# suutari/meterelf

Measured on AMD Instinct MI355X. Metric: frames/sec (640x480), full pipeline, digits identical to the oracle, higher is better.
Workload: dtype u8; 1 GPU; Batch=1024 per GPU, full pipeline incl. TM_CCOEFF match + needle reading, 4 dials/frame, sample-images1 params, frames 480x640 synthesised from the readable fixtures (shift +-8, noise sigma 2), 4 distinct batches in rotation (3.77 GB of frames per GPU); global_batch=1024, parallelism=dp1, frames_read_ok_batch0=1023

## Files before the change

### meterelf_amd/csrc/k_match_mfma.hip

```cpp
#include <limits.h>
#include <stdio.h>
#include <stdlib.h>
#include <string.h>

#include <algorithm>

#include "melf_device.h"
#include <hip/hip_ext.h>

#include "melf_internal.h"

namespace melf {

typedef int i32x4 __attribute__((ext_vector_type(4)));
typedef int i32x8 __attribute__((ext_vector_type(8)));
typedef int i32x16 __attribute__((ext_vector_type(16)));

typedef unsigned int u32x4m __attribute__((ext_vector_type(4)));

typedef uint32_t u32x4a4 __attribute__((ext_vector_type(4), aligned(4)));
template <bool FROM_BGR>
__global__ __launch_bounds__(256) void k_prep_lplane(MatchSrc src, int nframes, int nkb, int rows_pad, int tw, int rwp, int pairs,
                                                     int8_t* __restrict__ Lg, uint16_t* __restrict__ R)
{
    constexpr int PX = FROM_BGR ? 3 : 1;
#include "prep_lplane_body.inc"
}

__global__ __launch_bounds__(256) void k_lplane_px4(MatchSrc src, int nframes, int nkb, int rows_pad, int tw, int rwp, int pairs,
                                                    int8_t* __restrict__ Lg, uint16_t* __restrict__ R)
{
    constexpr int PX = 4;
#include "prep_lplane_body.inc"
}

struct MfmaGeom {
    int rh, rw;
    int rows_pad;
    int th_pad;
    int nframes;
    int nparts;
    int na;
    int k1;
    int rows, th;
    int ntiles;
    double tmean;
};

#ifdef MELF_MATCH_STAMP
__device__ uint64_t g_match_stamps[4 * 8192];
__device__ uint64_t g_match_loop_end[8192];
extern "C" __attribute__((visibility("default"))) int melf_debug_match_stamps(uint64_t* out, int nwaves)
{
    return hipMemcpyFromSymbol(out, HIP_SYMBOL(g_match_stamps), sizeof(uint64_t) * 4 * (size_t)(nwaves < 8192 ? nwaves : 8192)) == hipSuccess ? 0 : -1;
}
extern "C" __attribute__((visibility("default"))) int melf_debug_match_loop_end(uint64_t* out, int nwaves)
{
    return hipMemcpyFromSymbol(out, HIP_SYMBOL(g_match_loop_end), sizeof(uint64_t) * (size_t)(nwaves < 8192 ? nwaves : 8192)) == hipSuccess ? 0 : -1;
}
#endif

__device__ inline bool better_m(float v, int i, float bv, int bi)
{
    return i != INT_MAX && (bi == INT_MAX || v > bv || (v == bv && i < bi));
}

template <int R, int NXB, int KS>
struct SliceLds {
    uint32_t acc[R * NXB][16][64];
    uint32_t wsa[32][64];
};

constexpr int MM_NF_DEV = 8;
template <int ND, int NXB, int R, int PD , int MFIRST, int MLAST, int KS = 1>
__device__ __forceinline__ void match_wave(const int8_t* __restrict__ Lg, const int8_t* __restrict__ Atab,
                                           const uint32_t* __restrict__ ws, const MfmaGeom& g,
                                           float* __restrict__ result_map, MatchPartial* __restrict__ partials,
                                           int grp, int rblk, int y0, void* lds_raw = nullptr)
{
    auto on = [](int r, int xb) -> bool {
        return r == 0 ? ((MFIRST >> xb) & 1) : (r == R - 1 ? ((MLAST >> xb) & 1) : true);
    };
    constexpr int NKB = ND + NXB - 1;
    constexpr int NBUF = R + PD;
    static_assert(PD == 1, "the template fragments are single-buffered: the next row's fragment d is requested right after this row's last use of fragment d");
    const int lane = threadIdx.x & 63;
    const int ks = KS > 1 ? __builtin_amdgcn_readfirstlane((int)(threadIdx.x >> 6)) : 0;
    const int SL = g.th_pad / KS, i_lo = ks * SL, i_hi = i_lo + SL;
    auto mine = [&](int r) -> bool { return KS == 1 || (r * KS) / R == ks; };
    SliceLds<R, NXB, KS>* const X = (SliceLds<R, NXB, KS>*)lds_raw;
    if (KS > 1) {
        uint32_t* z = (uint32_t*)X;
        for (int i = threadIdx.x; i < (int)(sizeof(SliceLds<R, NXB, KS>) / 4); i += 64 * KS) z[i] = 0;
        __syncthreads();
    }

    const uint32_t l16 = (uint32_t)lane * 16u;
    const __amdgpu_buffer_rsrc_t rsL = __builtin_amdgcn_make_buffer_rsrc(const_cast<int8_t*>(Lg + (size_t)grp * g.rows_pad * (size_t)NKB * 1024), 0,
                                                                         (int)((unsigned)g.rows_pad * (unsigned)NKB * 1024u), 0x27000);
    const __amdgpu_buffer_rsrc_t rsA = __builtin_amdgcn_make_buffer_rsrc(const_cast<int8_t*>(Atab + 1024), 0, (int)((unsigned)(g.th_pad + PD) * MM_NF_DEV * 1024u), 0x27000);
    const unsigned rsR_bytes = (unsigned)g.rows * 4096u;
    const __amdgpu_buffer_rsrc_t rsR = __builtin_amdgcn_make_buffer_rsrc(const_cast<uint32_t*>(ws + (size_t)grp * g.rows * 1024), 0, (int)rsR_bytes, 0x27000);
    auto LD = [&](__amdgpu_buffer_rsrc_t rs, unsigned rowoff, int slot) -> i32x4 {
        return __builtin_amdgcn_raw_buffer_load_b128(rs, l16, rowoff + (unsigned)slot * 1024u, 0);
    };
    const unsigned Lrow = (unsigned)y0 * (unsigned)NKB * 1024u;
    const int idxP = ((const int*)Atab)[lane];
    const int idxLo = 0x44444444, idxHi = (int)0xEEEEEEEEu;
    constexpr unsigned ROWB = (unsigned)NKB * 1024u;
    constexpr unsigned AROWB = (unsigned)MM_NF_DEV * 1024u;
    constexpr int NP = NXB;
    constexpr int NKD = NKB - 2 * NP;
    static_assert(ND == 7 && (NXB == 1 || NXB == 2), "the sub-block schedule below is written out for 7 Toeplitz blocks");

    i32x16 acc[R][NXB];
#pragma unroll
    for (int r = 0; r < R; ++r)
#pragma unroll
        for (int xb = 0; xb < NXB; ++xb)
#pragma unroll
            for (int e = 0; e < 16; ++e) acc[r][xb][e] = 0;

    constexpr int PERIOD = NBUF;
    const int istart = i_lo + (((SL - y0 % SL) % SL) / PERIOD) * PERIOD;
    i32x8 pp[NBUF][NP];
    i32x4 kd[NBUF][NKD];
    i32x4 a06, ad[5], a1s, a5s;
    uint32_t wsa[32];
    i32x4 rwv[4];
    auto rw_row = [&](int i) -> unsigned {
        return i < g.th ? (unsigned)min(y0 + i, g.rows - 1) * 4096u : rsR_bytes;
    };
    auto load_pp = [&](i32x8& d, unsigned row, int slot) {
        const i32x4 lo = LD(rsL, row, slot), hi = LD(rsL, row, slot + 1);
        d = __builtin_shufflevector(lo, hi, 0, 1, 2, 3, 4, 5, 6, 7);
    };
    auto SP = [&](int r, int xb, const i32x4& a, const i32x8& b, int idx) {
        if (on(r, xb)) acc[r][xb] = __builtin_amdgcn_smfmac_i32_32x32x64_i8(a, b, acc[r][xb], idx, 0, 0);
    };
    auto DN = [&](int r, int xb, const i32x4& a, const i32x4& b) {
        if (on(r, xb)) acc[r][xb] = __builtin_amdgcn_mfma_i32_32x32x32_i8(a, b, acc[r][xb], 0, 0, 0);
    };
    constexpr int NM1_0 = R - ((MFIRST & 1) == 0) - ((MLAST & 1) == 0);
    constexpr int NM1_1 = NXB == 2 ? R - ((MFIRST & 2) == 0) - ((MLAST & 2) == 0) : 0;
    constexpr int NM2 = NM1_0 + NM1_1;
#pragma unroll
    for (int j = 0; j < 32; ++j) wsa[j] = 0;
    auto ws_add = [&](int p) {
#pragma unroll
        for (int c = 0; c < 4; ++c) {
            const uint32_t v = (uint32_t)rwv[p][c];
            wsa[8 * p + 2 * c] += v & 0xffffu;
            wsa[8 * p + 2 * c + 1] += v >> 16;
            asm("" : "+v"(wsa[8 * p + 2 * c]));
            asm("" : "+v"(wsa[8 * p + 2 * c + 1]));
        }
    };
#define MELF_SGB(MFMAS, VALUS) __builtin_amdgcn_sched_group_barrier(0x008, MFMAS, 0); __builtin_amdgcn_sched_group_barrier(0x002, VALUS, 0);
#define MELF_SPREAD(NM) \
    if constexpr ((NM) >= 8) { MELF_SGB(1, 1) MELF_SGB(1, 1) MELF_SGB(1, 1) MELF_SGB(1, 1) MELF_SGB(1, 1) MELF_SGB(1, 1) MELF_SGB(1, 1) MELF_SGB(1, 1) } \
    else if constexpr ((NM) >= 4) { MELF_SGB(1, 2) MELF_SGB(1, 2) MELF_SGB(1, 2) MELF_SGB(1, 2) } \
    else { MELF_SGB(1, 4) MELF_SGB(1, 4) }
#define MELF_FENCE __builtin_amdgcn_sched_barrier(0);
#define MELF_LOAD1 __builtin_amdgcn_sched_group_barrier(0x008, 1, 0); __builtin_amdgcn_sched_group_barrier(0x020, 1, 0);
#define MELF_LOADS1 MELF_LOAD1
#define MELF_LOADS2 MELF_LOAD1 MELF_LOAD1
#define MELF_LOADS3 MELF_LOAD1 MELF_LOAD1 MELF_LOAD1
    for (int phase = 0; phase < 2; ++phase) {
        const int ibeg = phase == 0 ? istart : i_lo, iend = phase == 0 ? i_hi : istart;
        if (ibeg >= iend) continue;
#pragma unroll
        for (int r = 0; r < NBUF - 1; ++r) {
            const unsigned row = Lrow + (unsigned)(ibeg + r) * ROWB;
#pragma unroll
            for (int p = 0; p < NP; ++p) load_pp(pp[r][p], row, 2 * p);
#pragma unroll
            for (int c = 0; c < NKD; ++c) kd[r][c] = LD(rsL, row, 2 * NP + c);
        }
        {
            const unsigned an = (unsigned)ibeg * AROWB;
            a06 = LD(rsA, an, 0);
#pragma unroll
            for (int d = 0; d < 5; ++d) ad[d] = LD(rsA, an, 1 + d);
            if constexpr (NXB == 2) { a1s = LD(rsA, an, 6); a5s = LD(rsA, an, 7); }
            const unsigned rp = rw_row(ibeg);
#pragma unroll
            for (int k = 0; k < 4; ++k) rwv[k] = LD(rsR, rp, k);
        }
        for (int i0 = ibeg; i0 < iend; i0 += PERIOD) {
#pragma unroll
            for (int s = 0; s < PERIOD; ++s) {
                const int i = i0 + s;
                const unsigned rowin = Lrow + (unsigned)(i + NBUF - 1) * ROWB;
                const unsigned an = (unsigned)(i + 1) * AROWB;
                const unsigned rwn = rw_row(i + 1);
                const int inc = (s + NBUF - 1) % NBUF;
#define CUR(r) ((s + (r)) % NBUF)
                if constexpr (NXB == 2) {
                    const unsigned rowinp = rowin - ROWB, anc = (unsigned)i * AROWB;
                    const int incp = (s + NBUF - 2) % NBUF;
                    MELF_FENCE
                    ad[4] = LD(rsA, anc, 5);
                    kd[incp][3] = LD(rsL, rowinp, 7);
#pragma unroll
                    for (int r = 0; r < R; ++r) { SP(r, 0, a06, pp[CUR(r)][0], idxP); SP(r, 1, a06, pp[CUR(r)][1], idxP); }
                    ws_add(0);
                    MELF_LOADS2 MELF_SPREAD(NM2 - 2)
                    MELF_FENCE
                    a06 = LD(rsA, an, 0);
                    rwv[0] = LD(rsR, rwn, 0);
#pragma unroll
                    for (int r = 0; r < R; ++r) SP(r, 1, a5s, pp[CUR(r)][0], idxHi);
                    MELF_LOADS2
                    MELF_FENCE
                    a5s = LD(rsA, an, 7);
                    load_pp(pp[inc][0], rowin, 0);
#pragma unroll
                    for (int r = 0; r < R; ++r) SP(r, 0, a1s, pp[CUR(r)][1], idxLo);
                    MELF_LOADS3
                    MELF_FENCE
                    a1s = LD(rsA, an, 6);
                    load_pp(pp[inc][1], rowin, 2);
#pragma unroll
                    for (int r = 0; r < R; ++r) DN(r, 1, ad[0], kd[CUR(r)][0]);
                    MELF_LOADS3
#pragma unroll
                    for (int q = 0; q < 3; ++q) {
                        MELF_FENCE
                        ad[q] = LD(rsA, an, 1 + q);
                        if (q >= 1) { kd[inc][q - 1] = LD(rsL, rowin, 4 + q - 1); rwv[q] = LD(rsR, rwn, q); }
#pragma unroll
                        for (int r = 0; r < R; ++r) { DN(r, 0, ad[1 + q], kd[CUR(r)][q]); DN(r, 1, ad[1 + q], kd[CUR(r)][q + 1]); }
                        ws_add(1 + q);
                        if (q >= 1) { MELF_LOADS3 MELF_SPREAD(NM2 - 3) } else { MELF_LOADS1 MELF_SPREAD(NM2 - 1) }
                    }
                    MELF_FENCE
                    ad[3] = LD(rsA, an, 4);
                    kd[inc][2] = LD(rsL, rowin, 6);
                    rwv[3] = LD(rsR, rwn, 3);
#pragma unroll
                    for (int r = 0; r < R; ++r) DN(r, 0, ad[4], kd[CUR(r)][3]);
                    MELF_LOADS3
                    MELF_FENCE
                } else {
                    MELF_FENCE
#pragma unroll
                    for (int r = 0; r < R; ++r) SP(r, 0, a06, pp[CUR(r)][0], idxP);
                    ws_add(0);
                    MELF_SPREAD(NM1_0)
                    MELF_FENCE
                    a06 = LD(rsA, an, 0);
#pragma unroll
                    for (int d = 0; d < 5; ++d) {
                        if (d == 0) load_pp(pp[inc][0], rowin, 0);
                        else kd[inc][d - 1] = LD(rsL, rowin, 2 + d - 1);
                        if (d < 4) rwv[d] = LD(rsR, rwn, d);
                        MELF_FENCE
#pragma unroll
                        for (int r = 0; r < R; ++r) DN(r, 0, ad[d], kd[CUR(r)][d]);
                        if (d < 3) { ws_add(1 + d); MELF_SPREAD(NM1_0) }
                        MELF_FENCE
                        ad[d] = LD(rsA, an, 1 + d);
                    }
                    kd[inc][4] = LD(rsL, rowin, 6);
                    MELF_FENCE
                }
#undef CUR
            }
        }
    }
#undef MELF_SGB
#undef MELF_SPREAD
#undef MELF_FENCE
#undef MELF_LOAD1
#undef MELF_LOADS1
#undef MELF_LOADS2
#undef MELF_LOADS3

#ifdef MELF_MATCH_STAMP
    if (threadIdx.x == 0 && blockIdx.x < 8192) g_match_loop_end[blockIdx.x] = __builtin_amdgcn_s_memtime();
#endif
    if constexpr (KS > 1) {
#pragma unroll
        for (int j = 0; j < 32; ++j) __hip_atomic_fetch_add(&X->wsa[j][lane], wsa[j], __ATOMIC_RELAXED, __HIP_MEMORY_SCOPE_WORKGROUP);
#pragma unroll
        for (int r = 0; r < R; ++r)
#pragma unroll
            for (int xb = 0; xb < NXB; ++xb) {
                if (!on(r, xb)) continue;
                if (!mine(r)) {
#pragma unroll
                    for (int e = 0; e < 16; ++e)
                        __hip_atomic_fetch_add(&X->acc[r * NXB + xb][e][lane], (uint32_t)acc[r][xb][e], __ATOMIC_RELAXED, __HIP_MEMORY_SCOPE_WORKGROUP);
                }
            }
        __syncthreads();
#pragma unroll
        for (int j = 0; j < 32; ++j) wsa[j] = X->wsa[j][lane];
#pragma unroll
        for (int r = 0; r < R; ++r)
#pragma unroll
            for (int xb = 0; xb < NXB; ++xb) {
                if (!on(r, xb)) continue;
                if (mine(r)) {
#pragma unroll
                    for (int e = 0; e < 16; ++e) acc[r][xb][e] += (int)X->acc[r * NXB + xb][e][lane];
                }
            }
    }
    const int n = lane & 31, hh = lane >> 5;
    const int f = grp * 32 + n;
    const bool lane_ok = f < g.nframes;
    float bestv = -INFINITY;
    int bestc = -1;
    i32x4 slide[2][4];
    auto slide_load = [&](int r) {
        const unsigned rout = (unsigned)min(y0 + r - 1, g.rows - 1) * 4096u;
        const unsigned rin = (unsigned)min(y0 + r - 1 + g.th, g.rows - 1) * 4096u;
#pragma unroll
        for (int k = 0; k < 4; ++k) { slide[0][k] = LD(rsR, rout, k); slide[1][k] = LD(rsR, rin, k); }
    };
#pragma unroll
    for (int r = 0; r < R; ++r) {
        if (r > 0) {
#pragma unroll
            for (int k = 0; k < 4; ++k)
#pragma unroll
                for (int c = 0; c < 4; ++c) {
                    const uint32_t a0 = (uint32_t)slide[1][k][c], b0 = (uint32_t)slide[0][k][c];
                    wsa[8 * k + 2 * c] += (a0 & 0xffffu) - (b0 & 0xffffu);
                    wsa[8 * k + 2 * c + 1] += (a0 >> 16) - (b0 >> 16);
                }
        }
        if (r + 1 < R) slide_load(r + 1);
        __builtin_amdgcn_sched_barrier(0);
        if (!mine(r)) continue;
        const int y = y0 + r;
        if (y >= g.rh) continue;
        float v[NXB][16];
#pragma unroll
        for (int xb = 0; xb < NXB; ++xb)
#pragma unroll
            for (int e = 0; e < 16; ++e) {
                if (!on(r, xb)) continue;
                const uint32_t wsv = wsa[16 * xb + e];
                const uint32_t cc = (uint32_t)acc[r][xb][e] + 128u * wsv + (uint32_t)g.k1;
                double num = (double)cc;
                num -= (double)wsv * g.tmean;
                v[xb][e] = (float)num;
            }
#pragma unroll
        for (int xb = 0; xb < NXB; ++xb) {
            if (!on(r, xb) || 32 * xb + 32 <= g.rw) continue;
#pragma unroll
            for (int e = 0; e < 16; ++e)
                if (32 * xb + (e & 3) + 8 * (e >> 2) + 4 * hh >= g.rw) v[xb][e] = -INFINITY;
        }
#pragma unroll
        for (int xb = 0; xb < NXB; ++xb)
#pragma unroll
            for (int e = 0; e < 16; ++e) {
                if (!on(r, xb)) continue;
                if (v[xb][e] > bestv) { bestv = v[xb][e]; bestc = (r * NXB + xb) * 16 + e; }
            }
        if (result_map) {
            float* mrow = result_map + (size_t)f * g.rh * g.rw + (size_t)y * g.rw;
#pragma unroll
            for (int xb = 0; xb < NXB; ++xb)
#pragma unroll
                for (int e = 0; e < 16; ++e) {
                    if (!on(r, xb)) continue;
                    const int x = 32 * xb + (e & 3) + 8 * (e >> 2) + 4 * hh;
                    if (lane_ok && x < g.rw) mrow[x] = v[xb][e];
                }
        }
        __builtin_amdgcn_sched_barrier(0);
    }
    int besti = INT_MAX;
    if (bestc >= 0) {
        const int e = bestc & 15, xb = (bestc >> 4) % NXB, r = (bestc >> 4) / NXB;
        besti = (y0 + r) * g.rw + 32 * xb + (e & 3) + 8 * (e >> 2) + 4 * hh;
    }
    {
        const float ov = __shfl_xor(bestv, 32, 64);
        const int oi = __shfl_xor(besti, 32, 64);
        if (better_m(ov, oi, bestv, besti)) { bestv = ov; besti = oi; }
    }
    if (lane < 32 && f < g.nframes) {
        MatchPartial p;
        p.val = bestv;
        p.idx = besti;
        partials[(size_t)f * g.nparts + rblk * KS + ks] = p;
    }
}


template <int ND, int NXB, int RB, int PD, int KS>
__device__ __forceinline__ void match_block(const int8_t* __restrict__ Lg, const int8_t* __restrict__ Atab,
                                            const uint32_t* __restrict__ ws, const MfmaGeom& g,
                                            float* __restrict__ result_map, MatchPartial* __restrict__ partials, void* lds)
{
    const int nblk = gridDim.x;
    const int id = blockIdx.x;
#ifdef MELF_MATCH_STAMP
    const uint64_t st_clk = __builtin_amdgcn_s_memtime(), st_rt = __builtin_amdgcn_s_memrealtime();
#endif
    const int per = nblk / 8, rem = nblk % 8, xcd = id & 7, sub = id >> 3;
    const int vid = (xcd < rem ? xcd * (per + 1) : rem * (per + 1) + (xcd - rem) * per) + sub;
    const int grp = vid / g.ntiles, rblk = vid - grp * g.ntiles;
    if (NXB == 2 && RB < 5 && rblk >= g.na) {
        const int q = rblk - g.na, base = RB * g.na + (2 * RB + 1) * (q >> 1);
        if ((q & 1) == 0) match_wave<ND, 2, (RB < 5 ? RB + 1 : RB), PD, 3, 1, KS>(Lg, Atab, ws, g, result_map, partials, grp, rblk, base, lds);
        else match_wave<ND, 2, (RB < 5 ? RB + 1 : RB), PD, 2, 3, KS>(Lg, Atab, ws, g, result_map, partials, grp, rblk, base + RB, lds);
    } else {
        match_wave<ND, NXB, RB, PD, 3, 3, KS>(Lg, Atab, ws, g, result_map, partials, grp, rblk, rblk * RB, lds);
    }
#ifdef MELF_MATCH_STAMP
    if (threadIdx.x == 0 && id < 8192) {
        g_match_stamps[4 * id + 0] = st_clk; g_match_stamps[4 * id + 1] = __builtin_amdgcn_s_memtime();
        g_match_stamps[4 * id + 2] = st_rt;  g_match_stamps[4 * id + 3] = __builtin_amdgcn_s_memrealtime();
    }
#endif
}

template <int ND, int NXB, int RB, int PD, int KS = 1>
__global__ __launch_bounds__(64 * KS, 1) void k_match_mfma(const int8_t* __restrict__ Lg, const int8_t* __restrict__ Atab,
                                                           const uint32_t* __restrict__ ws, MfmaGeom g,
                                                           float* __restrict__ result_map, MatchPartial* __restrict__ partials)
{
    if constexpr (NXB == 2 && RB >= 4) asm volatile("" ::: "a199");
    if constexpr (KS > 1) {
        __shared__ __attribute__((aligned(16))) SliceLds<(NXB == 2 && RB < 5 ? RB + 1 : RB), NXB, KS> lds;
        match_block<ND, NXB, RB, PD, KS>(Lg, Atab, ws, g, result_map, partials, &lds);
    } else {
        match_block<ND, NXB, RB, PD, 1>(Lg, Atab, ws, g, result_map, partials, nullptr);
    }
}
constexpr int MM_ND = 7, MM_PD = 1;
constexpr int MM_NF = 8;
static int round_up(int v, int m) { return (v + m - 1) / m * m; }
static int mm_th_pad(int th, int rb, bool pairs, int ks = 1)
{
    static const int lcm2[6] = {0, 0, 12, 20, 30, 6};
    return ks * round_up((th + ks - 1) / ks, pairs ? lcm2[rb] : rb + 1);
}
static int mm_th_pad_max(int th) { return std::max(round_up(th, 60), std::max(mm_th_pad(th, 4, true, 2), mm_th_pad(th, 4, true, 4))); }

bool mfma_match_ok(int th, int tw, int rows, int cols)
{
    const int rh = rows - th + 1, rw = cols - tw + 1;
    const int nd = (tw + 31 + 31) / 32;
    return rh >= 1 && rw >= 1 && rw <= 64 && nd == MM_ND && tw <= 32 * (MM_ND - 1) && cols <= 32 * (MM_ND + (rw > 32 ? 2 : 1) - 1) &&
           (long)th * tw * 65025L < (1L << 32);
}

static double mm_wave_cycles(int R, int units, int nxb, int th_pad, int ks = 1)
{
    const int nkb = MM_ND + nxb - 1;
    const int nf = nxb == 2 ? 8 : 6;
    const double load = R >= 4 ? 7.0 : (R == 3 ? 17.0 : 30.0);
    return (double)(th_pad / ks) * ((double)units * (MM_ND - 1) * 32.0 + (double)(nkb + nf + 4) * load) + (double)((units + ks - 1) / ks) * 1300.0 + 4000.0 + R * 300.0 +
           (ks > 1 ? 6000.0 : 0.0);
}

MfmaPlan mfma_plan(int th, int tw, int rows, int cols, int nframes)
{
    MfmaPlan p = {};
    p.rh = rows - th + 1;
    p.rw = cols - tw + 1;
    p.nxb = p.rw > 32 ? 2 : 1;
    p.nkb = MM_ND + p.nxb - 1;
    p.groups = (nframes + 31) / 32;
    const int simds = 1024;
    int force_rb = 0, force_np = -1, force_ks = 0;
    if (const char* e = getenv("MELF_MATCH_LAYOUT")) {
        if (sscanf(e, "%d,%d,%d", &force_rb, &force_np, &force_ks) < 1 || force_rb < 2 || force_rb > 5) { force_rb = 0; force_np = -1; force_ks = 0; }
        if (force_ks != 1 && force_ks != 2 && force_ks != 4) force_ks = force_rb ? 1 : 0;
        if (force_ks > 1 && force_rb != 4) force_ks = 1;
    }
    double best = 0;
    p.rb = 0;
    p.ks = 1;
    for (int ks = 1; ks <= 4; ks *= 2) {
        if (force_ks && ks != force_ks) continue;
        for (int rb = 2; rb <= 5; ++rb) {
            if (force_rb && rb != force_rb) continue;
            if (ks > 1 && rb != 4) continue;
            const int np_max = (p.nxb == 2 && rb < 5) ? (p.rh + 2 * rb) / (2 * rb + 1) : 0;
            auto waves_of = [&](int np) -> long {
                const int rest = p.rh - (2 * rb + 1) * np;
                return (long)((rest > 0 ? (rest + rb - 1) / rb : 0) + 2 * np) * p.groups * ks;
            };
            long rounds_min = LONG_MAX;
            for (int np = 0; np <= np_max; ++np) rounds_min = std::min(rounds_min, (waves_of(np) + simds - 1) / simds);
            int np_few = 0;
            while (np_few < np_max && (waves_of(np_few) + simds - 1) / simds > rounds_min) ++np_few;
            for (int np = 0; np <= np_max; ++np) {
                if (force_np >= 0) { if (np != std::min(force_np, np_max)) continue; }
                else if (np != 0 && np != np_few) continue;
                const int rest = p.rh - (2 * rb + 1) * np;
                const int na = rest > 0 ? (rest + rb - 1) / rb : 0;
                const long waves = (long)(na + 2 * np) * p.groups * ks;
                const long rounds = (waves + simds - 1) / simds;
                const int th_pad = mm_th_pad(th, rb, np > 0, ks);
                const int upr = p.nxb;
                const double w_full = mm_wave_cycles(rb, upr * rb, p.nxb, th_pad, ks), w_pair = mm_wave_cycles(rb + 1, upr * rb + 1, p.nxb, th_pad, ks);
                const double longest = np > 0 ? w_pair : w_full;
                const double total = (double)p.groups * ks * ((double)na * w_full + 2.0 * np * w_pair);
                const double w_avg = total / (double)std::max<long>(waves, 1);
                const long full = waves / simds, part = waves - full * simds;
                const double cost = (double)full * 1.5 * w_avg + (part > 0 ? std::max(longest, 1.5 * (double)part * w_avg / simds) : 0.0);
                (void)rounds;
                if (!p.rb || cost < best * 0.98) {
                    best = cost;
                    p.rb = rb; p.na = na; p.np = np; p.th_pad = th_pad; p.ks = ks;
                }
            }
        }
    }
    p.ntiles = p.na + 2 * p.np;
    p.nparts = p.ntiles * p.ks;
    const int rows_cov = p.rb * p.na + (2 * p.rb + 1) * p.np;
    p.rows_pad = rows_cov + p.th_pad + MM_PD + 1;
    p.lg_bytes = (size_t)p.groups * p.rows_pad * p.nkb * 1024;
    p.r_bytes = (size_t)p.groups * rows * 64 * 32 * sizeof(uint16_t);
    return p;
}

size_t mfma_atab_bytes(int th)
{
    return 1024 + (size_t)(mm_th_pad_max(th) + MM_PD) * MM_NF * 1024;
}

void mfma_build_atab(const uint8_t* templ, int th, int tw, int8_t* atab)
{
    const int th_pad = mm_th_pad_max(th);
    uint32_t* idx = (uint32_t*)atab;
    memset(atab, 0, 1024);
    int8_t* fr = atab + 1024;
    auto cand_cols = [&](int m, int hA, int ja, int cols[4]) {
        const int hB = ja >> 3, t = 4 * hA + ((ja >> 1) & 3), k0 = 16 * hB + 2 * t;
        cols[0] = k0 - m; cols[1] = k0 + 1 - m; cols[2] = 32 * (MM_ND - 1) + k0 - m; cols[3] = cols[2] + 1;
        return k0;
    };
    int pos[64][16];
    for (int l = 0; l < 64; ++l)
        for (int ja = 0; ja < 16; ja += 2) {
            int cols[4], cand[4], nc = 0;
            cand_cols(l & 31, l >> 5, ja, cols);
            for (int v = 0; v < 4; ++v) if (cols[v] >= 0 && cols[v] < tw) cand[nc++] = v;
            if (nc > 2) { fprintf(stderr, "[melf] mfma_build_atab: template of %d columns does not pair up\n", tw); abort(); }
            int v0 = 0, v1 = 1;
            if (nc == 2) { v0 = cand[0]; v1 = cand[1]; }
            else if (nc == 1) { v0 = cand[0] < 3 ? cand[0] : 0; v1 = 3; }
            pos[l][ja] = v0; pos[l][ja + 1] = v1;
            idx[l] |= ((uint32_t)v0 << (2 * ja)) | ((uint32_t)v1 << (2 * ja + 2));
        }
    for (int i = 0; i < th_pad + MM_PD; ++i) {
        auto Tq = [&](int col) -> int8_t { return (i < th && col >= 0 && col < tw) ? (int8_t)((int)templ[(size_t)i * tw + col] - 128) : (int8_t)0; };
        int8_t* row = fr + (size_t)i * MM_NF * 1024;
        for (int l = 0; l < 64; ++l) {
            const int m = l & 31, hA = l >> 5;
            for (int d = 1; d <= 5; ++d)
                for (int j = 0; j < 16; ++j) row[((size_t)d * 64 + l) * 16 + j] = Tq(32 * d + 16 * hA + j - m);
            for (int ja = 0; ja < 16; ++ja) {
                int cols[4];
                const int k0 = cand_cols(m, hA, ja & ~1, cols);
                row[((size_t)0 * 64 + l) * 16 + ja] = Tq(cols[pos[l][ja]]);
                row[((size_t)6 * 64 + l) * 16 + ja] = Tq(32 * 1 + k0 + (ja & 1) - m);
                row[((size_t)7 * 64 + l) * 16 + ja] = Tq(32 * 5 + k0 + (ja & 1) - m);
            }
        }
    }
}

void launch_match_prep(const MatchSrc& src, int pix, int n, int groups, int rows_pad, int nkb, int rwp, int tw, int8_t* d_lg,
                       uint16_t* d_r, hipStream_t stream, int pairs)
{
    dim3 grid(rows_pad, groups), block(256);
    const size_t pre_bytes = (size_t)32 * (nkb * 32 + 8) * sizeof(int16_t);
    int dev = 0;
    (void)hipGetDevice(&dev);
    static bool attr_set[64] = {false};
    if (dev >= 0 && dev < 64 && !attr_set[dev]) {
        (void)hipFuncSetAttribute((const void*)k_prep_lplane<true>, hipFuncAttributeMaxDynamicSharedMemorySize, 128 * 1024);
        (void)hipFuncSetAttribute((const void*)k_prep_lplane<false>, hipFuncAttributeMaxDynamicSharedMemorySize, 128 * 1024);
        (void)hipFuncSetAttribute((const void*)k_lplane_px4, hipFuncAttributeMaxDynamicSharedMemorySize, 128 * 1024);
        attr_set[dev] = true;
    }
    if (pix == PIX_PLANE) hipLaunchKernelGGL((k_prep_lplane<false>), grid, block, pre_bytes, stream, src, n, nkb, rows_pad, tw, rwp, pairs, d_lg, d_r);
    else if (pix_bytes(pix) == 4) hipLaunchKernelGGL(k_lplane_px4, grid, block, pre_bytes, stream, src, n, nkb, rows_pad, tw, rwp, pairs, d_lg, d_r);
    else hipLaunchKernelGGL((k_prep_lplane<true>), grid, block, pre_bytes, stream, src, n, nkb, rows_pad, tw, rwp, pairs, d_lg, d_r);
}

void launch_mfma_prep(const MatchSrc& src, int pix, int n, const MfmaPlan& p, int th, int tw, int8_t* d_lg,
                      uint16_t* d_r, hipStream_t stream)
{
    (void)th;
    launch_match_prep(src, pix, n, p.groups, p.rows_pad, p.nkb, 64, tw, d_lg, d_r, stream, p.nxb);
}

template <int NXB, int RB, int KS>
static void launch_mm(dim3 grid, hipStream_t stream, hipEvent_t ev_start, hipEvent_t ev_stop, const int8_t* d_lg,
                      const int8_t* d_atab, const uint32_t* d_ws, const MfmaGeom& g, float* d_result_map, MatchPartial* d_partials)
{
    hipExtLaunchKernelGGL((k_match_mfma<MM_ND, NXB, RB, MM_PD, KS>), grid, dim3(64 * KS), 0, stream, ev_start, ev_stop, 0, d_lg, d_atab, d_ws, g,
                              d_result_map, d_partials);
}

void launch_mfma_match(int n, const MfmaPlan& p, int th, int tw, long tsum, double tmean, const int8_t* d_atab,
                       const int8_t* d_lg, const uint32_t* d_ws, float* d_result_map, MatchPartial* d_partials,
                       hipStream_t stream, hipEvent_t ev_start, hipEvent_t ev_stop)
{
    MfmaGeom g;
    g.rh = p.rh; g.rw = p.rw; g.rows_pad = p.rows_pad; g.th_pad = p.th_pad; g.nframes = n; g.nparts = p.nparts;
    g.na = p.na; g.ntiles = p.ntiles;
    g.k1 = (int)(128 * (tsum - 128L * th * tw));
    g.rows = p.rh + th - 1; g.th = th;
    g.tmean = tmean;
    dim3 grid(p.ntiles * p.groups);
#define MM_CASE(NXB_, RB_) \
    case NXB_ * 8 + RB_: launch_mm<NXB_, RB_, 1>(grid, stream, ev_start, ev_stop, d_lg, d_atab, d_ws, g, d_result_map, d_partials); break;
#define MM_CASE_KS(NXB_, KS_) \
    case 64 * KS_ + NXB_ * 8 + 4: launch_mm<NXB_, 4, KS_>(grid, stream, ev_start, ev_stop, d_lg, d_atab, d_ws, g, d_result_map, d_partials); break;
    switch ((p.ks > 1 ? 64 * p.ks : 0) + p.nxb * 8 + p.rb) {
        MM_CASE(1, 2) MM_CASE(1, 3) MM_CASE(1, 4) MM_CASE(1, 5)
        MM_CASE(2, 2) MM_CASE(2, 3) MM_CASE(2, 4) MM_CASE(2, 5)
        MM_CASE_KS(1, 2) MM_CASE_KS(2, 2) MM_CASE_KS(1, 4) MM_CASE_KS(2, 4)
        default:
            fprintf(stderr, "[melf] k_match_mfma: no instantiation for %d column blocks x %d rows per wave x %d K slices\n", p.nxb, p.rb, p.ks);
            abort();
    }
#undef MM_CASE
#undef MM_CASE_KS
}

}
```

### meterelf_amd/csrc/prep_lplane_body.inc

```
    constexpr int PB = PX == 4 ? 4 : 3;
    constexpr int WIN = PX == 4 ? 128 : 100;
    __shared__ __attribute__((aligned(16))) uint32_t tile[8 * 2 * 32 * 4];
    extern __shared__ int16_t pre_dyn[];
    const int pstride = nkb * 32 + 8;
    const int y = blockIdx.x, grp = blockIdx.y;
    const int t = threadIdx.x, n = t >> 3, kl = t & 7;
    const int f = grp * 32 + n;
    int carry = 0;
    const bool rows_safe = (size_t)min(grp * 32 + 31, nframes - 1) * src.frame_stride + (size_t)(src.y0 + y) * src.row_stride +
                           (size_t)(src.x0 + 32 * (nkb - 1)) * PB + WIN <= src.readable;
    u32x4m* out = (u32x4m*)(Lg + ((size_t)grp * rows_pad + y) * (size_t)nkb * 1024);
    for (int kc = 0; kc < nkb; kc += 8) {
        const int kb = kc + kl;
        uint32_t w[8] = {0, 0, 0, 0, 0, 0, 0, 0};
        const bool live = kb < nkb && f < nframes && y < src.rows && kb * 32 < src.cols;
        if (live) {
            const uint8_t* prow = src.base + (size_t)f * src.frame_stride + (size_t)(src.y0 + y) * src.row_stride;
            const int xbeg = kb * 32;
            const int npx = min(32, src.cols - xbeg);
            if (PX == 3) {
                const size_t o = (size_t)(src.x0 + xbeg) * 3;
                const uint8_t* p = prow + o;
                const int mis = (int)((size_t)p & 3);
                if (rows_safe || (size_t)f * src.frame_stride + (size_t)(src.y0 + y) * src.row_stride + o + 100 <= src.readable) {
                    const uint32_t* q = (const uint32_t*)(p - mis);
                    uint32_t d[25];
#pragma unroll
                    for (int i = 0; i < 25; ++i) d[i] = q[i];
                    uint32_t a[24];
#pragma unroll
                    for (int i = 0; i < 24; ++i) a[i] = __builtin_amdgcn_alignbit(d[i + 1], d[i], (uint32_t)mis * 8u);
#pragma unroll
                    for (int k = 0; k < 32; ++k) {
                        const int j = (3 * k) >> 2, sh = ((3 * k) & 3) * 8;
                        const uint32_t px = sh <= 8 ? (a[j] >> sh) : __builtin_amdgcn_alignbit(a[j + 1 < 24 ? j + 1 : 23], a[j], sh);
                        const int L = hls_lightness_fast(px & 255, (px >> 8) & 255, (px >> 16) & 255);
                        w[k >> 2] |= (uint32_t)((L - 128) & 255) << ((k & 3) * 8);
                    }
                } else {
                    for (int k = 0; k < npx; ++k) {
                        const int L = hls_lightness(p[3 * k], p[3 * k + 1], p[3 * k + 2]);
                        w[k >> 2] |= (uint32_t)((L - 128) & 255) << ((k & 3) * 8);
                    }
                }
            } else if (PX == 4) {
                const size_t o = (size_t)(src.x0 + xbeg) * 4;
                const uint8_t* p = prow + o;
                if (rows_safe || (size_t)f * src.frame_stride + (size_t)(src.y0 + y) * src.row_stride + o + 128 <= src.readable) {
                    const u32x4a4* q = (const u32x4a4*)p;
                    u32x4a4 d[8];
#pragma unroll
                    for (int i = 0; i < 8; ++i) d[i] = q[i];
#pragma unroll
                    for (int k = 0; k < 32; ++k) {
                        const uint32_t px = d[k >> 2][k & 3];
                        const int L = hls_lightness_fast(px & 255, (px >> 8) & 255, (px >> 16) & 255);
                        w[k >> 2] |= (uint32_t)((L - 128) & 255) << ((k & 3) * 8);
                    }
                } else {
                    for (int k = 0; k < npx; ++k) {
                        const uint32_t px = ((const uint32_t*)p)[k];
                        const int L = hls_lightness(px & 255, (px >> 8) & 255, (px >> 16) & 255);
                        w[k >> 2] |= (uint32_t)((L - 128) & 255) << ((k & 3) * 8);
                    }
                }
            } else {
                const uint8_t* p = prow + src.x0 + xbeg;
                for (int k = 0; k < npx; ++k) w[k >> 2] |= (uint32_t)(((int)p[k] - 128) & 255) << ((k & 3) * 8);
            }
        }
        if (kc) __syncthreads();
#pragma unroll
        for (int h = 0; h < 2; ++h) {
            u32x4m v = {w[4 * h], w[4 * h + 1], w[4 * h + 2], w[4 * h + 3]};
            *(u32x4m*)(tile + ((kl * 2 + h) * 32 + n) * 4) = v;
        }
        int run = 0;
#pragma unroll
        for (int j = 0; j < 8; ++j) run = __builtin_amdgcn_sdot4((int)w[j], 0x01010101, run, false);
        int off = run;
#pragma unroll
        for (int dlt = 1; dlt < 8; dlt <<= 1) {
            const int o2 = __shfl_up(off, dlt, 8);
            if (kl >= dlt) off += o2;
        }
        const int chunk_total = __shfl(off, 7, 8);
        off += carry - run;
        carry += chunk_total;
        if (kb < nkb) {
            int acc = off;
#pragma unroll
            for (int k = 0; k < 32; k += 2) {
                acc += (int)(int8_t)((w[k >> 2] >> ((k & 3) * 8)) & 255u);
                const uint32_t lo16 = (uint32_t)acc & 0xffffu;
                acc += (int)(int8_t)((w[k >> 2] >> (((k + 1) & 3) * 8)) & 255u);
                *(uint32_t*)&pre_dyn[n * pstride + kb * 32 + k] = lo16 | ((uint32_t)acc << 16);
            }
        }
        __syncthreads();
        const int nb = min(8, nkb - kc);
        if (pairs == 0) {
            for (int i = t; i < nb * 64; i += 256) out[kc * 64 + i] = *(const u32x4m*)(tile + i * 4);
        } else {
            for (int i = t; i < nb * 64; i += 256) {
                const int slot = i >> 6, li = i & 63;
                u32x4m v;
                if (slot < 2 * pairs) {
                    const int p = slot >> 1, hl = slot & 1;
                    const uint2 lo2 = *(const uint2*)(tile + (p * 64 + li) * 4 + 2 * hl), hi2 = *(const uint2*)(tile + ((p + 6) * 64 + li) * 4 + 2 * hl);
                    v.x = __builtin_amdgcn_perm(hi2.x, lo2.x, 0x05040100u); v.y = __builtin_amdgcn_perm(hi2.x, lo2.x, 0x07060302u);
                    v.z = __builtin_amdgcn_perm(hi2.y, lo2.y, 0x05040100u); v.w = __builtin_amdgcn_perm(hi2.y, lo2.y, 0x07060302u);
                } else {
                    v = *(const u32x4m*)(tile + ((slot - pairs) * 64 + li) * 4);
                }
                out[i] = v;
            }
        }
    }
    if (y < src.rows) {
        uint16_t* ro = R + (((size_t)grp * src.rows + y) * rwp) * 32;
        const int bias = tw * 128;
        const int pmax = nkb * 32 - 1;
        const int ln = t & 63, nn = ln & 31, hh = ln >> 5;
        for (int kk = t >> 6; kk < rwp / 16; kk += 4) {
            const int xb = kk >> 1, e0 = 8 * (kk & 1);
            uint32_t o[4];
#pragma unroll
            for (int q = 0; q < 8; ++q) {
                const int e = e0 + q;
                const int x = 32 * xb + (e & 3) + 8 * (e >> 2) + 4 * hh;
                const int hi = (int)pre_dyn[nn * pstride + min(x + tw - 1, pmax)], lo = x > 0 ? (int)pre_dyn[nn * pstride + min(x - 1, pmax)] : 0;
                const uint32_t v = (uint32_t)(hi - lo + bias) & 0xffffu;
                if (q & 1) o[q >> 1] |= v << 16; else o[q >> 1] = v;
            }
            u32x4m ov = {o[0], o[1], o[2], o[3]};
            *(u32x4m*)(ro + ((size_t)kk * 64 + ln) * 8) = ov;
        }
    }
```

Baseline: 4.241 million frames/s.

## Compact prep-kernel prefix-sum LDS to needed blocks and cap VGPRs

The prep kernel now keeps only the row prefix-sum blocks that are later read: the low blocks used for the left edge and the high blocks used for the right edge. These are packed into a smaller dynamic shared-memory buffer with remapped indices, which shrinks LDS per block. The prep kernels are also capped at 32 VGPRs. Both changes aim at higher occupancy for the LDS- and register-limited preprocessing kernel, at the risk of register spills in the heavily unrolled BGR path.

New measurement: 4.226 million frames/s (median of 2 runs). Within noise of the previous version (-0.3%).

```diff
diff --git a/meterelf_amd/csrc/k_match_mfma.hip b/meterelf_amd/csrc/k_match_mfma.hip
--- a/meterelf_amd/csrc/k_match_mfma.hip
+++ b/meterelf_amd/csrc/k_match_mfma.hip
@@ -19,15 +19,28 @@
 typedef unsigned int u32x4m __attribute__((ext_vector_type(4)));
 
 typedef uint32_t u32x4a4 __attribute__((ext_vector_type(4), aligned(4)));
+struct PrepPrefix {
+    int lo_blk, hb_blk, hi_blk, stride;
+};
+__host__ __device__ inline PrepPrefix prep_prefix_layout(int nkb, int tw, int rwp)
+{
+    if (rwp % 32 == 0 && tw >= 1 && tw <= nkb * 32) {
+        const int lo_blk = rwp / 32, hb_blk = (tw - 1) / 32;
+        const int hi_blk = min(nkb, (tw - 1 + rwp - 1) / 32 + 1) - hb_blk;
+        if (hb_blk >= lo_blk && lo_blk + hi_blk < nkb) return PrepPrefix{lo_blk, hb_blk, hi_blk, (lo_blk + hi_blk) * 32 + 8};
+    }
+    return PrepPrefix{nkb, nkb, 0, nkb * 32 + 8};
+}
+constexpr int PREP_VGPRS = 32;
 template <bool FROM_BGR>
-__global__ __launch_bounds__(256) void k_prep_lplane(MatchSrc src, int nframes, int nkb, int rows_pad, int tw, int rwp, int pairs,
+__global__ __launch_bounds__(256) __attribute__((amdgpu_num_vgpr(PREP_VGPRS))) void k_prep_lplane(MatchSrc src, int nframes, int nkb, int rows_pad, int tw, int rwp, int pairs,
                                                      int8_t* __restrict__ Lg, uint16_t* __restrict__ R)
 {
     constexpr int PX = FROM_BGR ? 3 : 1;
 #include "prep_lplane_body.inc"
 }
 
-__global__ __launch_bounds__(256) void k_lplane_px4(MatchSrc src, int nframes, int nkb, int rows_pad, int tw, int rwp, int pairs,
+__global__ __launch_bounds__(256) __attribute__((amdgpu_num_vgpr(PREP_VGPRS))) void k_lplane_px4(MatchSrc src, int nframes, int nkb, int rows_pad, int tw, int rwp, int pairs,
                                                     int8_t* __restrict__ Lg, uint16_t* __restrict__ R)
 {
     constexpr int PX = 4;
@@ -578,7 +591,7 @@
                        uint16_t* d_r, hipStream_t stream, int pairs)
 {
     dim3 grid(rows_pad, groups), block(256);
-    const size_t pre_bytes = (size_t)32 * (nkb * 32 + 8) * sizeof(int16_t);
+    const size_t pre_bytes = (size_t)32 * prep_prefix_layout(nkb, tw, rwp).stride * sizeof(int16_t);
     int dev = 0;
     (void)hipGetDevice(&dev);
     static bool attr_set[64] = {false};
diff --git a/meterelf_amd/csrc/prep_lplane_body.inc b/meterelf_amd/csrc/prep_lplane_body.inc
--- a/meterelf_amd/csrc/prep_lplane_body.inc
+++ b/meterelf_amd/csrc/prep_lplane_body.inc
@@ -2,7 +2,8 @@
     constexpr int WIN = PX == 4 ? 128 : 100;
     __shared__ __attribute__((aligned(16))) uint32_t tile[8 * 2 * 32 * 4];
     extern __shared__ int16_t pre_dyn[];
-    const int pstride = nkb * 32 + 8;
+    const PrepPrefix pl = prep_prefix_layout(nkb, tw, rwp);
+    const int pstride = pl.stride, hi_base = 32 * (pl.lo_blk - pl.hb_blk);
     const int y = blockIdx.x, grp = blockIdx.y;
     const int t = threadIdx.x, n = t >> 3, kl = t & 7;
     const int f = grp * 32 + n;
@@ -87,14 +88,16 @@
         const int chunk_total = __shfl(off, 7, 8);
         off += carry - run;
         carry += chunk_total;
-        if (kb < nkb) {
+        const bool keep = kb < pl.lo_blk || (unsigned)(kb - pl.hb_blk) < (unsigned)pl.hi_blk;
+        if (keep) {
+            const int kb_dst = kb < pl.lo_blk ? kb : kb - pl.hb_blk + pl.lo_blk;
             int acc = off;
 #pragma unroll
             for (int k = 0; k < 32; k += 2) {
                 acc += (int)(int8_t)((w[k >> 2] >> ((k & 3) * 8)) & 255u);
                 const uint32_t lo16 = (uint32_t)acc & 0xffffu;
                 acc += (int)(int8_t)((w[k >> 2] >> (((k + 1) & 3) * 8)) & 255u);
-                *(uint32_t*)&pre_dyn[n * pstride + kb * 32 + k] = lo16 | ((uint32_t)acc << 16);
+                *(uint32_t*)&pre_dyn[n * pstride + kb_dst * 32 + k] = lo16 | ((uint32_t)acc << 16);
             }
         }
         __syncthreads();
@@ -129,7 +132,7 @@
             for (int q = 0; q < 8; ++q) {
                 const int e = e0 + q;
                 const int x = 32 * xb + (e & 3) + 8 * (e >> 2) + 4 * hh;
-                const int hi = (int)pre_dyn[nn * pstride + min(x + tw - 1, pmax)], lo = x > 0 ? (int)pre_dyn[nn * pstride + min(x - 1, pmax)] : 0;
+                const int hi = (int)pre_dyn[nn * pstride + min(x + tw - 1, pmax) + hi_base], lo = x > 0 ? (int)pre_dyn[nn * pstride + min(x - 1, pmax)] : 0;
                 const uint32_t v = (uint32_t)(hi - lo + bias) & 0xffffu;
                 if (q & 1) o[q >> 1] |= v << 16; else o[q >> 1] = v;
             }
```
